# tobwei/APTAI

Measured on AMD Instinct MI355X. Metric: utterances/sec (10 s @ 16 kHz) train-step, higher is better.
Workload: dtype bf16

## Files before the change

### aptai_amd/csrc/common.h

```cpp
#pragma once
#include <hip/hip_runtime.h>
#include <stdint.h>
#include <stdio.h>
#include <string.h>

#include "../../include/aptai_hip.h"

typedef uint16_t bf16_t;

typedef __attribute__((ext_vector_type(8))) __bf16 bf16x8;
typedef __attribute__((ext_vector_type(4))) __bf16 bf16x4;
typedef __attribute__((ext_vector_type(4))) short short4v;
typedef __attribute__((ext_vector_type(8))) short short8v;
typedef __attribute__((ext_vector_type(4))) float f32x4;
typedef __attribute__((ext_vector_type(16))) float f32x16;
typedef __attribute__((ext_vector_type(2))) uint32_t u32x2;
typedef __attribute__((ext_vector_type(4))) uint32_t u32x4;

#define LDS_PTR(p) ((__attribute__((address_space(3))) void*)(p))
#define GLB_PTR(p) ((const __attribute__((address_space(1))) void*)(p))

void aptai_set_error(const char* fmt, ...);
const uint32_t* aptai_seed_salt(const void* stream);
const int32_t* aptai_frame_bounds(const void* stream);
#define APTAI_FAIL(code, ...)            \
    do {                                 \
        aptai_set_error(__VA_ARGS__);    \
        return (code);                   \
    } while (0)
#define APTAI_REQUIRE(cond, ...)                                   \
    do {                                                           \
        if (!(cond)) APTAI_FAIL(APTAI_ERR_INVALID, __VA_ARGS__);   \
    } while (0)
#define APTAI_LAUNCH(...)             \
    do {                              \
        (void)hipGetLastError();      \
        hipLaunchKernelGGL(__VA_ARGS__); \
    } while (0)
#define APTAI_CHECK_LAUNCH(name)                                                          \
    do {                                                                                  \
        hipError_t e__ = hipGetLastError();                                               \
        if (e__ != hipSuccess) APTAI_FAIL(APTAI_ERR_LAUNCH, "%s: %s", name, hipGetErrorString(e__)); \
    } while (0)

__device__ __forceinline__ float bf2f(bf16_t v) { return __uint_as_float(((uint32_t)v) << 16); }
__device__ __forceinline__ bf16_t f2bf(float f) {
    __bf16 b = (__bf16)f;
    return __builtin_bit_cast(bf16_t, b);
}
__device__ __forceinline__ uint32_t pack2bf(float lo, float hi) {
    typedef __bf16 bf2_t __attribute__((ext_vector_type(2)));
    typedef float f2_t __attribute__((ext_vector_type(2)));
    const f2_t v = {lo, hi};
    return __builtin_bit_cast(uint32_t, __builtin_convertvector(v, bf2_t));
}
__device__ __forceinline__ float lo_bf(uint32_t v) { return __uint_as_float(v << 16); }
__device__ __forceinline__ float hi_bf(uint32_t v) { return __uint_as_float(v & 0xffff0000u); }

__device__ __forceinline__ float wave_sum(float v) {
#pragma unroll
    for (int o = 32; o > 0; o >>= 1) v += __shfl_xor(v, o, 64);
    return v;
}
__device__ __forceinline__ float wave_max(float v) {
#pragma unroll
    for (int o = 32; o > 0; o >>= 1) v = fmaxf(v, __shfl_xor(v, o, 64));
    return v;
}

__device__ __forceinline__ float fast_exp2(float x) { return __builtin_amdgcn_exp2f(x); }
__device__ __forceinline__ float fast_log2(float x) { return __builtin_amdgcn_logf(x); }
__device__ __forceinline__ float gelu_erf(float x) { return 0.5f * x * (1.0f + erff(x * 0.70710678118654752f)); }
__device__ __forceinline__ float gelu_erf_grad(float x) {
    const float cdf = 0.5f * (1.0f + erff(x * 0.70710678118654752f));
    const float pdf = 0.39894228040143268f * __expf(-0.5f * x * x);
// ... 82 lines not shown
```

### aptai_amd/csrc/conv.hip

```cpp
#include <stdlib.h>

#include "common.h"

namespace {

constexpr int C0 = 512, KW = 10, STRIDE = 5;
constexpr int FRAMES_PER_BLOCK_STATS = 256;

struct Conv0Args {
    const float* audio; long S;
    const float* w; const float* bias; const float* gamma; const float* beta;
    bf16_t* out;
    int B, T_real, T_alloc;
    float eps;
    float* partials;
    const float* stats;
    int nchunks;
    const int* bounds;
};

__device__ __forceinline__ int frames_collated(const int* __restrict__ bounds, int T_real) {
    if (bounds == nullptr) return T_real;
    const int tb = bounds[0];
    return tb < 1 ? 1 : (tb < T_real ? tb : T_real);
// ... 95 lines not shown

template <bool LENS>
__global__ __launch_bounds__(256) void conv0_moments_kernel(const float* __restrict__ audio, long S, int T_static,
                                                            float* __restrict__ partials, int nch, const int* __restrict__ bounds,
                                                            const int* __restrict__ lens) {
    const int b = blockIdx.y, chunk = blockIdx.x;
    const int T_real = LENS ? frames_own(lens, b, bounds, T_static) : frames_collated(bounds, T_static);
    if (LENS && chunk * AC_FRAMES_PER_BLOCK >= T_real) return;
    __shared__ float red[4][AC_TERMS];
    const int lane = threadIdx.x & 63, wave = threadIdx.x >> 6;
    const float* xb = audio + (long)b * S;
    float acc[AC_TERMS];
#pragma unroll
    for (int i = 0; i < AC_TERMS; ++i) acc[i] = 0.f;
    const int t0 = chunk * AC_FRAMES_PER_BLOCK;
    int t1 = t0 + AC_FRAMES_PER_BLOCK;
    t1 = t1 < T_real ? t1 : T_real;
    for (int t = t0 + threadIdx.x; t < t1; t += 256) {
        float x[KW];
#pragma unroll
        for (int k = 0; k < KW; ++k) x[k] = xb[(long)t * STRIDE + k];
        int idx = KW;
#pragma unroll
        for (int k = 0; k < KW; ++k) {
            acc[k] += x[k];
#pragma unroll
            for (int k2 = k; k2 < KW; ++k2) { acc[idx] = fmaf(x[k], x[k2], acc[idx]); ++idx; }
        }
    }
#pragma unroll
    for (int i = 0; i < AC_TERMS; ++i) {
        const float v = wave_sum(acc[i]);
        if (lane == 0) red[wave][i] = v;
    }
    __syncthreads();
    if (threadIdx.x < AC_TERMS)
        partials[((long)b * nch + chunk) * AC_TERMS + threadIdx.x] =
            red[0][threadIdx.x] + red[1][threadIdx.x] + red[2][threadIdx.x] + red[3][threadIdx.x];
}

template <bool LENS>
__global__ void conv0_moments_final_kernel(const float* __restrict__ partials, const float* __restrict__ w,
                                           const float* __restrict__ bias, float* __restrict__ stats, int nch, int T_real,
                                           float eps, const int* __restrict__ bounds, const int* __restrict__ lens) {
    __shared__ double mom[AC_TERMS];
    const int b = blockIdx.x, c = threadIdx.x;
    const int frames = LENS ? frames_own(lens, b, bounds, T_real) : frames_collated(bounds, T_real);
    const int nsum = LENS ? (frames + AC_FRAMES_PER_BLOCK - 1) / AC_FRAMES_PER_BLOCK : nch;
    if (c < AC_TERMS) {
        double s = 0.0;
        for (int k = 0; k < nsum; ++k) s += (double)partials[((long)b * nch + k) * AC_TERMS + c];
        mom[c] = s / frames;
    }
    __syncthreads();
    double wk[KW];
#pragma unroll
    for (int k = 0; k < KW; ++k) wk[k] = (double)w[c * KW + k];
    const double bc = bias ? (double)bias[c] : 0.0;
    double wm = 0.0, q = 0.0;
    int idx = KW;
#pragma unroll
    for (int k = 0; k < KW; ++k) {
        wm += wk[k] * mom[k];
#pragma unroll
        for (int k2 = k; k2 < KW; ++k2) q += (k2 == k ? 1.0 : 2.0) * wk[k] * wk[k2] * mom[idx++];
    }
    const double mean = bc + wm;
    double var = q + 2.0 * bc * wm + bc * bc - mean * mean;
    var = var < 0.0 ? 0.0 : var;
    stats[((long)b * 2 + 0) * C0 + c] = (float)mean;
    stats[((long)b * 2 + 1) * C0 + c] = (float)(1.0 / sqrt(var + (double)eps));
}

typedef float f32x2 __attribute__((ext_vector_type(2)));

__device__ __forceinline__ f32x2 gelu_fast2(f32x2 x) {
    const f32x2 xc = {__builtin_amdgcn_fmed3f(x.x, -7.0f, 7.0f), __builtin_amdgcn_fmed3f(x.y, -7.0f, 7.0f)};
    const f32x2 x2 = xc * xc;
    f32x2 p = __builtin_elementwise_fma(x2, (f32x2){APTAI_GELU_A5 * APTAI_NLOG2E, APTAI_GELU_A5 * APTAI_NLOG2E},
                                        (f32x2){APTAI_GELU_A3 * APTAI_NLOG2E, APTAI_GELU_A3 * APTAI_NLOG2E});
    p = __builtin_elementwise_fma(p, x2, (f32x2){APTAI_GELU_A1 * APTAI_NLOG2E, APTAI_GELU_A1 * APTAI_NLOG2E});
    const f32x2 z = xc * p;
    const f32x2 e = (f32x2){__builtin_amdgcn_exp2f(z.x), __builtin_amdgcn_exp2f(z.y)} + (f32x2){1.0f, 1.0f};
    return x * (f32x2){__builtin_amdgcn_rcpf(e.x), __builtin_amdgcn_rcpf(e.y)};
}

template <bool LENS>
__global__ __launch_bounds__(256) void conv0_group_kernel(Conv0Args a, const int* __restrict__ lens) {
    const int lane = threadIdx.x & 63, wave = threadIdx.x >> 6;
    const int b = blockIdx.y;
    const int T_real = LENS ? frames_own(lens, b, a.bounds, a.T_real) : a.T_real;
    f32x2 w2[4][KW], b2[4];
    {
        float w[8][KW], bias[8];
        load_weights(a, lane, w, bias);
#pragma unroll
        for (int j = 0; j < 8; ++j) {
            const int c = lane * 8 + j;
            const float mu = a.stats[((long)b * 2 + 0) * C0 + c], rs = a.stats[((long)b * 2 + 1) * C0 + c];
            const float sc = rs * a.gamma[c];
            const float sh = fmaf(bias[j] - mu, sc, a.beta[c]);
#pragma unroll
            for (int k = 0; k < KW; ++k) w2[j >> 1][k][j & 1] = w[j][k] * sc;
            b2[j >> 1][j & 1] = sh;
        }
    }
// ... 612 lines not shown
        float v = t < T_real ? g[t * KW + r] : 0.f;
        if (t >= 1 && t - 1 < T_real) v += g[(t - 1) * KW + r + STRIDE];
        daudio[(long)b * S + s] = v;
    }
}

bool conv0_bwd_mfma() {
    static const bool on = !(getenv("APTAI_CONV0_BWD_MFMA") && atoi(getenv("APTAI_CONV0_BWD_MFMA")) == 0);
    return on;
}

}

extern "C" int64_t aptai_conv0_workspace_bytes(int64_t B, int64_t T_real) {
    const long nchunks = ceil_div(T_real, FRAMES_PER_BLOCK_STATS);
    return (B * nchunks * 2 * C0 + B * 2 * C0) * 4;
}

template <bool LENS>
static int conv0_fwd_impl(const char* who, const float* audio, int64_t B, int64_t S, const float* weight, const float* bias,
                          const float* gamma, const float* beta, int mode, float eps, void* out, int64_t T_real, int64_t T_alloc,
                          int64_t C, int64_t Kw, int64_t stride, void* workspace, float* stats_out, const int32_t* lens,
                          void* stream_) {
    hipStream_t stream = (hipStream_t)stream_;
    APTAI_REQUIRE(audio && weight && gamma && beta && out, "%s: null pointer", who);
    APTAI_REQUIRE(!LENS || lens, "%s: null frame_lens0", who);
    APTAI_REQUIRE(C == C0 && Kw == KW && stride == STRIDE, "%s: built for C=512, k=10, s=5 (got %ld,%ld,%ld)", who,
                  (long)C, (long)Kw, (long)stride);
    APTAI_REQUIRE(B > 0 && T_real > 0 && T_alloc >= T_real, "%s: bad frame counts", who);
    APTAI_REQUIRE((T_real - 1) * STRIDE + KW <= S, "%s: T_real=%ld frames need more than S=%ld samples", who, (long)T_real, (long)S);
    APTAI_REQUIRE(mode == 0 || mode == 1, "%s: mode must be 0 (group) or 1 (layer)", who);
    const int* bounds = (const int*)aptai_frame_bounds(stream_);
    Conv0Args a;
    memset(&a, 0, sizeof(a));
    a.audio = audio; a.S = S; a.w = weight; a.bias = bias; a.gamma = gamma; a.beta = beta;
    a.out = (bf16_t*)out; a.B = (int)B; a.T_real = (int)T_real; a.T_alloc = (int)T_alloc; a.eps = eps;
    if (LENS) a.bounds = bounds;
    long blocks = ceil_div(T_alloc, 4 * 8);
    if (blocks > 1024) blocks = 1024;
    if (mode == 1) {
        APTAI_LAUNCH(conv0_layer_kernel<LENS>, dim3((unsigned)blocks, (unsigned)B), dim3(256), 0, stream, a, (const int*)lens);
        APTAI_CHECK_LAUNCH("conv0_layer_kernel");
        return APTAI_OK;
    }
    APTAI_REQUIRE(workspace != nullptr, "%s: group mode needs a workspace", who);
    a.nchunks = (int)ceil_div(T_real, FRAMES_PER_BLOCK_STATS);
    a.partials = (float*)workspace;
    float* stats = stats_out ? stats_out : (float*)workspace + (long)B * a.nchunks * 2 * C0;
    a.stats = stats;
    const int nch = (int)ceil_div(T_real, AC_FRAMES_PER_BLOCK);
    APTAI_LAUNCH(conv0_moments_kernel<LENS>, dim3((unsigned)nch, (unsigned)B), dim3(256), 0, stream, audio, (long)S, (int)T_real,
                 a.partials, nch, bounds, (const int*)lens);
    APTAI_CHECK_LAUNCH("conv0_moments_kernel");
    APTAI_LAUNCH(conv0_moments_final_kernel<LENS>, dim3((unsigned)B), dim3(C0), 0, stream, (const float*)a.partials, weight, bias,
                 stats, nch, (int)T_real, eps, bounds, (const int*)lens);
    APTAI_CHECK_LAUNCH("conv0_moments_final_kernel");
    static int use_mfma = -1;
    if (use_mfma < 0) {
        const char* e = getenv("APTAI_CONV0_MFMA");
        use_mfma = e ? atoi(e) : 1;
    }
    if (use_mfma && T_alloc % 16 == 0) {
        long mb = ceil_div(1536, B);
        const long mb_max = ceil_div(T_alloc / 16, 4);
        if (mb > mb_max) mb = mb_max;
        APTAI_LAUNCH(conv0_group_mfma_kernel<LENS>, dim3((unsigned)mb, (unsigned)B), dim3(256), 0, stream, a, (const int*)lens);
        APTAI_CHECK_LAUNCH("conv0_group_mfma_kernel");
        return APTAI_OK;
    }
    APTAI_LAUNCH(conv0_group_kernel<LENS>, dim3((unsigned)blocks, (unsigned)B), dim3(256), 0, stream, a, (const int*)lens);
    APTAI_CHECK_LAUNCH("conv0_group_kernel");
    return APTAI_OK;
}

extern "C" int aptai_conv0_fwd(const float* audio, int64_t B, int64_t S, const float* weight, const float* bias,
                               const float* gamma, const float* beta, int mode, float eps, void* out, int64_t T_real,
                               int64_t T_alloc, int64_t C, int64_t Kw, int64_t stride, void* workspace, float* stats_out,
                               void* stream_) {
    return conv0_fwd_impl<false>("aptai_conv0_fwd", audio, B, S, weight, bias, gamma, beta, mode, eps, out, T_real, T_alloc, C, Kw, stride,
                                 workspace, stats_out, nullptr, stream_);
}

extern "C" int aptai_conv0_fwd_lens(const float* audio, int64_t B, int64_t S, const float* weight, const float* bias,
                                    const float* gamma, const float* beta, int mode, float eps, void* out, int64_t T_real,
                                    int64_t T_alloc, int64_t C, int64_t Kw, int64_t stride, void* workspace, float* stats_out,
                                    const int32_t* frame_lens0, void* stream_) {
    return conv0_fwd_impl<true>("aptai_conv0_fwd_lens", audio, B, S, weight, bias, gamma, beta, mode, eps, out, T_real, T_alloc, C, Kw,
                                stride, workspace, stats_out, frame_lens0, stream_);
}

extern "C" int64_t aptai_conv0_bwd_workspace_bytes(int64_t B, int64_t T_real) {
    const long nch = ceil_div(T_real, BWD_FRAMES_PER_BLOCK);
    return (B * nch * 2 * C0 + B * 2 * C0 + B * nch * C0 * 13) * 4;
}

extern "C" int aptai_conv0_bwd(const float* audio, int64_t B, int64_t S, const float* weight, const float* bias, const float* gamma,
                               const float* beta, int mode, float eps, const void* dy, int64_t T_real, int64_t T_alloc,
                               const float* fwd_stats, float* dweight, float* dbias, float* dgamma, float* dbeta, void* workspace,
                               void* stream_) {
    hipStream_t stream = (hipStream_t)stream_;
    APTAI_REQUIRE(audio && weight && gamma && beta && dy && dweight && workspace, "aptai_conv0_bwd: null pointer");
    APTAI_REQUIRE(mode == 0 || mode == 1, "aptai_conv0_bwd: mode");
    APTAI_REQUIRE(mode == 1 || fwd_stats, "aptai_conv0_bwd: group mode needs the forward statistics");
    APTAI_REQUIRE((T_real - 1) * STRIDE + KW <= S && T_alloc >= T_real, "aptai_conv0_bwd: bad frame counts");
    Conv0BwdArgs a;
    memset(&a, 0, sizeof(a));
    a.f.audio = audio; a.f.S = S; a.f.w = weight; a.f.bias = bias; a.f.gamma = gamma; a.f.beta = beta; a.f.B = (int)B;
    a.f.T_real = (int)T_real; a.f.T_alloc = (int)T_alloc; a.f.eps = eps; a.f.stats = fwd_stats;
// ... 76 lines not shown
```

### aptai_amd/csrc/elementwise.hip

```cpp
#include "common.h"

namespace {

__global__ void cast_f32_bf16_kernel(const float* __restrict__ src, bf16_t* __restrict__ dst, long n4) {
    const long stride = (long)gridDim.x * blockDim.x;
    for (long i = (long)blockIdx.x * blockDim.x + threadIdx.x; i < n4; i += stride) {
        const f32x4 v = ((const f32x4*)src)[i];
        ((u32x2*)dst)[i] = (u32x2){pack2bf(v[0], v[1]), pack2bf(v[2], v[3])};
    }
}

__global__ void cast_multi_kernel(const int64_t* __restrict__ table) {
    const int64_t* job = table + (long)blockIdx.y * 4;
    const long n = job[2];
    const long base = (long)blockIdx.x * 8192;
    if (base >= n) return;
    const float* src = (const float*)job[0];
    const bool copy = job[3] != 0;
#pragma unroll
    for (int it = 0; it < 4; ++it) {
        const long i = base + (long)(it * 256 + threadIdx.x) * 8;
        if (i >= n) break;
        const f32x4 a = *(const f32x4*)(src + i), b = *(const f32x4*)(src + i + 4);
        if (copy) {
// ... 88 lines not shown
        const int a = i / Kw, kk = i % Kw;
        const long src = dgrad ? (((long)(grp * Cg + a) * Cg + r) * Kw + kk) : ((long)row * n + i);
        slab[a * (Kw + 1) + kk] = v[src] * gain[kk] / norm[kk];
    }
    __syncthreads();
    bf16_t* out = (dgrad ? wd : wf) + (long)row * n;
    for (int j = threadIdx.x; j < n; j += 256) {
        const int kk = j / Cg, a = j % Cg;
        out[j] = f2bf(slab[a * (Kw + 1) + (dgrad ? Kw - 1 - kk : kk)]);
    }
}

__global__ __launch_bounds__(256) void posconv_wn_dot_kernel(const float* __restrict__ dwf, const float* __restrict__ v,
                                                             float* __restrict__ partial, int Cg, int Kw) {
    extern __shared__ float slab[];
    __shared__ float red[256];
    const int o = blockIdx.x, n = Cg * Kw;
    for (int i = threadIdx.x; i < n; i += 256) slab[(i / Cg) * (Cg + 1) + i % Cg] = dwf[(long)o * n + i];
    __syncthreads();
    float s = 0.f;
    for (int i = threadIdx.x; i < n; i += 256) {
        const int c = i / Kw, kk = i % Kw;
        s = fmaf(slab[kk * (Cg + 1) + c], v[(long)o * n + i], s);
    }
    red[threadIdx.x] = s;
    __syncthreads();
    if ((int)threadIdx.x < Kw) {
        float t = 0.f;
        for (int j = threadIdx.x; j < 256; j += Kw) t += red[j];
        partial[(long)o * Kw + threadIdx.x] = t;
    }
}
__global__ __launch_bounds__(256) void posconv_wn_final_kernel(const float* __restrict__ partial, const float* __restrict__ norm,
                                                               float* __restrict__ dot, float* __restrict__ dgain, int H, int Kw) {
    __shared__ float red[256];
    const int kk = blockIdx.x;
    const float s = tap_total(partial, H, Kw, kk, red);
    if (threadIdx.x == 0) {
        dot[kk] = s;
        dgain[kk] = s / norm[kk];
    }
}
__global__ __launch_bounds__(256) void posconv_wn_apply_kernel(const float* __restrict__ dwf, const float* __restrict__ v,
                                                               const float* __restrict__ gain, const float* __restrict__ norm,
                                                               const float* __restrict__ dot, float* __restrict__ dv, int Cg, int Kw) {
    extern __shared__ float slab[];
    const int o = blockIdx.x, n = Cg * Kw;
    for (int i = threadIdx.x; i < n; i += 256) slab[(i / Cg) * (Cg + 1) + i % Cg] = dwf[(long)o * n + i];
    __syncthreads();
    for (int i = threadIdx.x; i < n; i += 256) {
        const int c = i / Kw, kk = i % Kw;
        const float nr = norm[kk];
        dv[(long)o * n + i] = gain[kk] / nr * (slab[kk * (Cg + 1) + c] - v[(long)o * n + i] * dot[kk] / (nr * nr));
    }
}

__global__ void posconv_pack_kernel(const bf16_t* __restrict__ x, const bf16_t* __restrict__ u, bf16_t* __restrict__ xg,
                                    bf16_t* __restrict__ rowmajor_out, int B, int Tp, int H, int Cg, int pad) {
    const long n4 = (long)B * Tp * H / 4;
    const long stride = (long)gridDim.x * blockDim.x;
    const int G = H / Cg;
    const long rows_p = Tp + 2 * pad;
    for (long i = (long)blockIdx.x * blockDim.x + threadIdx.x; i < n4; i += stride) {
        const long e = i * 4;
        const long row = e / H;
        const int col = (int)(e % H);
        u32x2 p = *(const u32x2*)(x + e);
        if (u) {
            const u32x2 q = *(const u32x2*)(u + e);
            p = (u32x2){pack2bf(lo_bf(p[0]) * gelu_fast_grad(lo_bf(q[0])), hi_bf(p[0]) * gelu_fast_grad(hi_bf(q[0]))),
                        pack2bf(lo_bf(p[1]) * gelu_fast_grad(lo_bf(q[1])), hi_bf(p[1]) * gelu_fast_grad(hi_bf(q[1])))};
            if (rowmajor_out) *(u32x2*)(rowmajor_out + e) = p;
        }
        const int grp = col / Cg, c = col % Cg;
        const long b = row / Tp, t = row % Tp;
        *(u32x2*)(xg + (((long)grp * B + b) * rows_p + pad + t) * Cg + c) = p;
    }
    (void)G;
}

constexpr int SPEC_MAX_SPANS = 256;
__device__ __forceinline__ uint32_t spec_rand(uint32_t ctr, uint32_t s0, uint32_t s1) { return rng_hash(ctr * 2654435761u + 12345u, s0, s1); }

__global__ __launch_bounds__(64) void spec_mask_kernel(const int* __restrict__ lens, uint8_t* __restrict__ mask, int T, float mask_prob,
                                                       int mask_length, int min_masks, uint32_t s0, uint32_t s1,
                                                       const uint32_t* __restrict__ salt) {
    __shared__ int starts[SPEC_MAX_SPANS];
    __shared__ int nspan_sh;
    apply_salt(salt, s0, s1);
    const int b = blockIdx.x, lane = threadIdx.x;
    uint8_t* row = mask + (long)b * T;
    for (int t = lane; t < T; t += 64) row[t] = 0;
    int len = lens[b];
    len = len < 0 ? 0 : (len > T ? T : len);
    if (lane == 0) {
        const float eps = (float)(spec_rand(0xE951u, s0, s1) >> 8) * (1.0f / 16777216.0f);
        int n = (int)(mask_prob * (float)len / (float)mask_length + eps);
        n = n > min_masks ? n : min_masks;
        if (n * mask_length > T) n = T / mask_length;
        const int range = len - (mask_length - 1);
        if (range < n) n = range > 0 ? range : 0;
        n = n < SPEC_MAX_SPANS ? n : SPEC_MAX_SPANS;
        for (int i = 0; i < n; ++i) {
            const int j = range - n + i;
            const int t = (int)(spec_rand((uint32_t)(b * SPEC_MAX_SPANS + i + 1), s0, s1) % (uint32_t)(j + 1));
            bool taken = false;
// ... 212 lines not shown
        keep_scales8(i * 8, s0, s1, thr_tv, sc_tv, mt);
        keep_scales8(i * 8, s0 ^ 0x5bd1e995u, s1, thr_ph, sc_ph, mp);
#pragma unroll
        for (int r = 0; r < 8; ++r) {
            const float th = tanh_fast(x[r] * mt[r]);
            g[r] = gt[r] * (1.f - th * th) * mt[r] + gp[r] * (x[r] * mp[r] > 0.f ? 1.f : 0.01f) * mp[r];
        }
        *(u32x4*)(dh + i * 8) = pack8f(g);
    }
    for (long i = (n8 << 3) + (long)blockIdx.x * blockDim.x + threadIdx.x; i < n; i += stride) {
        const float x = bf2f(h[i]);
        float xt = x, xp = x, mt = 1.f, mp = 1.f;
        if (thr_tv) { mt = drop_keep((uint64_t)i, s0, s1, thr_tv) ? sc_tv : 0.f; xt = x * mt; }
        if (thr_ph) { mp = drop_keep((uint64_t)i, s0 ^ 0x5bd1e995u, s1, thr_ph) ? sc_ph : 0.f; xp = x * mp; }
        const float th = tanh_fast(xt);
        dh[i] = f2bf(bf2f(d_tv[i]) * (1.f - th * th) * mt + bf2f(d_ph[i]) * (xp > 0.f ? 1.f : 0.01f) * mp);
    }
}

__global__ void dropout_kernel(const bf16_t* __restrict__ x, bf16_t* __restrict__ y, long n, uint32_t s0, uint32_t s1,
                               uint32_t thr, float sc, const uint32_t* __restrict__ salt) {
    apply_salt(salt, s0, s1);
    const long stride = (long)gridDim.x * blockDim.x;
    const long n8 = n >> 3;
    for (long i = (long)blockIdx.x * blockDim.x + threadIdx.x; i < n8; i += stride) {
        float v[8], m[8];
        unpack8(*(const u32x4*)(x + i * 8), v);
        keep_scales8(i * 8, s0, s1, thr, sc, m);
#pragma unroll
        for (int r = 0; r < 8; ++r) v[r] *= m[r];
        *(u32x4*)(y + i * 8) = pack8f(v);
    }
    for (long i = (n8 << 3) + (long)blockIdx.x * blockDim.x + threadIdx.x; i < n; i += stride)
        y[i] = drop_keep((uint64_t)i, s0, s1, thr) ? f2bf(bf2f(x[i]) * sc) : (bf16_t)0;
}

__global__ void dgelu_kernel(const bf16_t* __restrict__ dy, const bf16_t* __restrict__ u, bf16_t* __restrict__ out, long n8) {
    const long stride = (long)gridDim.x * blockDim.x;
    for (long i = (long)blockIdx.x * blockDim.x + threadIdx.x; i < n8; i += stride) {
        const u32x4 d = ((const u32x4*)dy)[i], x = ((const u32x4*)u)[i];
        u32x4 o;
#pragma unroll
        for (int r = 0; r < 4; ++r)
            o[r] = pack2bf(lo_bf(d[r]) * gelu_fast_grad(lo_bf(x[r])), hi_bf(d[r]) * gelu_fast_grad(hi_bf(x[r])));
        ((u32x4*)out)[i] = o;
    }
}

inline unsigned grid_for(long n, int block = 256, int max_blocks = 4096) {
    long b = ceil_div(n, block);
    return (unsigned)(b < 1 ? 1 : (b > max_blocks ? max_blocks : b));
}

}

extern "C" int aptai_cast_f32_to_bf16(const float* src, void* dst, int64_t rows, int64_t cols, int64_t ld_dst, void* stream) {
    APTAI_REQUIRE(src && dst && rows > 0 && cols > 0, "aptai_cast_f32_to_bf16: bad arguments");
    if (ld_dst == cols && (rows * cols) % 4 == 0 && ((uintptr_t)src % 16 == 0) && ((uintptr_t)dst % 8 == 0)) {
        const long n4 = rows * cols / 4;
        APTAI_LAUNCH(cast_f32_bf16_kernel, dim3(grid_for(n4)), dim3(256), 0, (hipStream_t)stream, src, (bf16_t*)dst, n4);
    } else {
        APTAI_LAUNCH(cast_rows_kernel, dim3(grid_for(rows * cols)), dim3(256), 0, (hipStream_t)stream, src,
                           (bf16_t*)dst, (long)rows, (long)cols, (long)ld_dst);
    }
    APTAI_CHECK_LAUNCH("cast kernel");
    return APTAI_OK;
}

extern "C" int aptai_cast_multi(const int64_t* table_dev, int64_t njobs, int64_t max_n, void* stream) {
    APTAI_REQUIRE(table_dev && njobs > 0 && njobs <= 65535 && max_n > 0, "aptai_cast_multi: bad arguments");
    const long chunks = ceil_div(max_n, 8192);
    APTAI_LAUNCH(cast_multi_kernel, dim3((unsigned)chunks, (unsigned)njobs), dim3(256), 0, (hipStream_t)stream, table_dev);
    APTAI_CHECK_LAUNCH("cast_multi_kernel");
    return APTAI_OK;
}

extern "C" int aptai_conv_weight_to_bf16(const float* src, void* dst, int64_t N, int64_t C, int64_t Kw, void* stream) {
    APTAI_REQUIRE(src && dst && N > 0 && C > 0 && Kw > 0, "aptai_conv_weight_to_bf16: bad arguments");
    APTAI_LAUNCH(conv_weight_kernel, dim3(grid_for(N * C * Kw)), dim3(256), 0, (hipStream_t)stream, src, (bf16_t*)dst,
                       (int)N, (int)C, (int)Kw);
    APTAI_CHECK_LAUNCH("conv_weight_kernel");
    return APTAI_OK;
}

extern "C" int aptai_posconv_weight(const float* v, const float* gain, float* norm_ws, void* w_fwd, void* w_dgrad,
                                    int64_t H, int64_t groups, int64_t Kw, void* stream) {
    APTAI_REQUIRE(v && gain && norm_ws && w_fwd, "aptai_posconv_weight: null pointer");
    APTAI_REQUIRE(groups > 0 && H % groups == 0 && (H / groups) % 8 == 0, "aptai_posconv_weight: H=%ld groups=%ld", (long)H, (long)groups);
    const int Cg = (int)(H / groups);
    APTAI_REQUIRE(Kw > 0 && 256 % Kw == 0, "aptai_posconv_weight: Kw=%ld must divide 256", (long)Kw);
    const long nel = (long)H * Cg * Kw;
    float* partial = norm_ws + Kw;
    APTAI_LAUNCH(posconv_norm_partial_kernel, dim3(PCN_BLOCKS), dim3(256), 0, (hipStream_t)stream, v, partial, nel, (int)Kw);
    APTAI_CHECK_LAUNCH("posconv_norm_partial_kernel");
    APTAI_LAUNCH(posconv_norm_final_kernel, dim3((unsigned)Kw), dim3(256), 0, (hipStream_t)stream, (const float*)partial, norm_ws, (int)Kw);
    APTAI_CHECK_LAUNCH("posconv_norm_final_kernel");
    const size_t slab_bytes = (size_t)Cg * (Kw + 1) * 4;
    APTAI_REQUIRE(slab_bytes <= 64 * 1024, "aptai_posconv_weight: Cg*Kw slab of %ld bytes exceeds the LDS budget", (long)slab_bytes);
    APTAI_LAUNCH(posconv_weight_kernel, dim3((unsigned)(w_dgrad ? 2 * H : H)), dim3(256), slab_bytes, (hipStream_t)stream, v, gain,
                       (const float*)norm_ws, (bf16_t*)w_fwd, (bf16_t*)w_dgrad, (int)H, Cg, (int)Kw);
    APTAI_CHECK_LAUNCH("posconv_weight_kernel");
    return APTAI_OK;
}

extern "C" int aptai_spec_augment_mask(const int32_t* frame_lens, void* mask_u8, int64_t B, int64_t T, float mask_prob, int64_t mask_length,
                                       int64_t min_masks, uint64_t seed, void* stream) {
    APTAI_REQUIRE(frame_lens && mask_u8 && B > 0 && T > 0, "aptai_spec_augment_mask: bad arguments");
    APTAI_REQUIRE(mask_length >= 1 && mask_length <= T, "aptai_spec_augment_mask: mask_length=%ld must lie in [1, T=%ld]", (long)mask_length, (long)T);
    APTAI_REQUIRE(mask_prob >= 0.f && mask_prob <= 1.f && min_masks >= 0, "aptai_spec_augment_mask: bad mask_prob / min_masks");
    APTAI_LAUNCH(spec_mask_kernel, dim3((unsigned)B), dim3(64), 0, (hipStream_t)stream, frame_lens, (uint8_t*)mask_u8, (int)T, mask_prob,
                 (int)mask_length, (int)min_masks, (uint32_t)seed, (uint32_t)(seed >> 32), aptai_seed_salt(stream));
    APTAI_CHECK_LAUNCH("spec_mask_kernel");
    return APTAI_OK;
}

extern "C" int aptai_posconv_weight_bwd(const float* dw_fwd, const float* v, const float* gain, const float* norm, float* dv, float* dgain,
                                       float* workspace, int64_t H, int64_t groups, int64_t Kw, void* stream) {
    APTAI_REQUIRE(dw_fwd && v && gain && norm && dv && dgain && workspace, "aptai_posconv_weight_bwd: null pointer");
    APTAI_REQUIRE(groups > 0 && H % groups == 0 && Kw > 0 && 256 % Kw == 0, "aptai_posconv_weight_bwd: H=%ld groups=%ld Kw=%ld", (long)H, (long)groups, (long)Kw);
    const int Cg = (int)(H / groups);
    const size_t slab_bytes = (size_t)Kw * (Cg + 1) * 4;
    APTAI_REQUIRE(slab_bytes <= 64 * 1024, "aptai_posconv_weight_bwd: slab of %ld bytes exceeds the LDS budget", (long)slab_bytes);
    float* partial = workspace;
    float* dot = workspace + H * Kw;
    hipStream_t st = (hipStream_t)stream;
    APTAI_LAUNCH(posconv_wn_dot_kernel, dim3((unsigned)H), dim3(256), slab_bytes, st, dw_fwd, v, partial, Cg, (int)Kw);
    APTAI_CHECK_LAUNCH("posconv_wn_dot_kernel");
    APTAI_LAUNCH(posconv_wn_final_kernel, dim3((unsigned)Kw), dim3(256), 0, st, (const float*)partial, norm, dot, dgain, (int)H, (int)Kw);
    APTAI_CHECK_LAUNCH("posconv_wn_final_kernel");
    APTAI_LAUNCH(posconv_wn_apply_kernel, dim3((unsigned)H), dim3(256), slab_bytes, st, dw_fwd, v, gain, norm, (const float*)dot, dv, Cg, (int)Kw);
    APTAI_CHECK_LAUNCH("posconv_wn_apply_kernel");
    return APTAI_OK;
}

extern "C" int aptai_posconv_pack(const void* x, const void* u, void* xg, void* rowmajor_out, int64_t B, int64_t Tp,
                                  int64_t H, int64_t groups, int64_t pad, void* stream) {
    APTAI_REQUIRE(x && xg, "aptai_posconv_pack: null pointer");
    APTAI_REQUIRE(groups > 0 && H % groups == 0 && (H / groups) % 4 == 0, "aptai_posconv_pack: H=%ld groups=%ld", (long)H, (long)groups);
    APTAI_LAUNCH(posconv_pack_kernel, dim3(grid_for(B * Tp * H / 4)), dim3(256), 0, (hipStream_t)stream,
                       (const bf16_t*)x, (const bf16_t*)u, (bf16_t*)xg, (bf16_t*)rowmajor_out, (int)B, (int)Tp, (int)H,
                       (int)(H / groups), (int)pad);
    APTAI_CHECK_LAUNCH("posconv_pack_kernel");
    return APTAI_OK;
}

static int frame_mask_fwd_impl(const char* who, void* h, const int32_t* lens, const uint8_t* spec_mask, const float* embed,
                               const uint8_t* feat_mask, int64_t B, int64_t Tp, int64_t T, int64_t H, void* stream) {
    APTAI_REQUIRE(h && lens && H % 4 == 0, "%s: bad arguments", who);
    APTAI_REQUIRE(!spec_mask || embed, "%s: spec mask without masked_spec_embed", who);
    APTAI_REQUIRE((uintptr_t)feat_mask % 4 == 0, "%s: feat_mask must be 4-byte aligned", who);
    const dim3 grid(grid_for(B * Tp * H / 4));
    if (feat_mask)
        APTAI_LAUNCH(frame_mask_kernel<true>, grid, dim3(256), 0, (hipStream_t)stream, (bf16_t*)h, lens, spec_mask, embed, feat_mask,
                     (int)B, (int)Tp, (int)T, (int)H);
    else
        APTAI_LAUNCH(frame_mask_kernel<false>, grid, dim3(256), 0, (hipStream_t)stream, (bf16_t*)h, lens, spec_mask, embed, feat_mask,
                     (int)B, (int)Tp, (int)T, (int)H);
    APTAI_CHECK_LAUNCH("frame_mask_kernel");
    return APTAI_OK;
}
extern "C" int aptai_frame_mask_fwd(void* h, const int32_t* lens, const uint8_t* spec_mask, const float* embed, int64_t B,
                                    int64_t Tp, int64_t T, int64_t H, void* stream) {
    return frame_mask_fwd_impl("aptai_frame_mask_fwd", h, lens, spec_mask, embed, nullptr, B, Tp, T, H, stream);
}
extern "C" int aptai_frame_feature_mask_fwd(void* h, const int32_t* lens, const uint8_t* spec_mask, const float* embed,
                                            const uint8_t* feat_mask, int64_t B, int64_t Tp, int64_t T, int64_t H, void* stream) {
    return frame_mask_fwd_impl("aptai_frame_feature_mask_fwd", h, lens, spec_mask, embed, feat_mask, B, Tp, T, H, stream);
}

static const int MASK_BWD_RPB = 32;
extern "C" int64_t aptai_frame_mask_bwd_workspace_bytes(int64_t B, int64_t Tp, int64_t H) {
    return ceil_div(B * Tp, MASK_BWD_RPB) * H * 4;
}
static int frame_mask_bwd_impl(const char* who, void* dy, const int32_t* lens, const uint8_t* spec_mask, const uint8_t* feat_mask,
                               float* dembed, void* workspace, int64_t B, int64_t Tp, int64_t T, int64_t H, void* stream) {
    APTAI_REQUIRE(dy && lens && H % 4 == 0, "%s: bad arguments", who);
    APTAI_REQUIRE((uintptr_t)feat_mask % 4 == 0, "%s: feat_mask must be 4-byte aligned", who);
    const long blocks = ceil_div(B * Tp, MASK_BWD_RPB);
    const bool want = spec_mask && dembed;
    APTAI_REQUIRE(!want || workspace, "%s: workspace needed for dembed", who);
    float* partials = want ? (float*)workspace : nullptr;
    if (feat_mask)
        APTAI_LAUNCH(frame_mask_bwd_kernel<true>, dim3((unsigned)blocks), dim3(256), 0, (hipStream_t)stream, (bf16_t*)dy, lens,
// ... 79 lines not shown
```

### aptai_amd/csrc/posconv.hip

```cpp
#include "common.h"

namespace {

constexpr int CG = 48, KW = 128, FR = 128;
constexpr int KTOT = KW * CG;
constexpr int XROWS = FR + KW - 1;
constexpr int X_BYTES = 6 * 256 * 16;
constexpr int W_STAGE = 512 * 16;

struct PosconvArgs {
    const bf16_t* xg; long x_group_stride, x_batch_stride;
    const bf16_t* w;
    const float* bias;
    const bf16_t* residual;
    bf16_t* out;
    bf16_t* out_pre;
    int Tp, H, gelu;
};

__device__ __forceinline__ void posconv_store(const PosconvArgs& a, const f32x4 accv, long row, int col) {
    float v[4] = {accv[0], accv[1], accv[2], accv[3]};
    if (a.bias) {
        const f32x4 bv = *(const f32x4*)(a.bias + col);
#pragma unroll
// ... 36 lines not shown
    }
    auto stage_w = [&](char* buf) {
#pragma unroll
        for (int it = 0; it < 2; ++it) {
            __builtin_amdgcn_global_load_lds(GLB_PTR(pw[it]), LDS_PTR(buf + (it * 256 + wave * 64) * 16), 16, 0, 0);
            pw[it] += 64;
        }
    };
    stage_w(sW);

    f32x4 acc[2][3];
#pragma unroll
    for (int i = 0; i < 2; ++i)
#pragma unroll
        for (int j = 0; j < 3; ++j) acc[i][j] = (f32x4){0.f, 0.f, 0.f, 0.f};

    const int a_off = (wave * 32 + (lane & 15)) * (CG * 2) + (lane >> 4) * 16;
    int b_off[3][2];
#pragma unroll
    for (int j = 0; j < 3; ++j)
#pragma unroll
        for (int ks = 0; ks < 2; ++ks) {
            const int row = j * 16 + (lane & 15), q = ks * 4 + (lane >> 4);
            b_off[j][ks] = row * 128 + ((q ^ (row & 7)) << 4);
        }

    constexpr int NKT = KTOT / 64;
    for (int kt = 0; kt < NKT; ++kt) {
        asm volatile("s_waitcnt vmcnt(0)" ::: "memory");
        __syncthreads();
        const int cur = kt & 1;
        if (kt + 1 < NKT) stage_w(sW + (cur ^ 1) * W_STAGE);
        const char* sw = sW + cur * W_STAGE;
        const char* sa = sX + a_off + kt * 128;
        bf16x8 af[2][2], bfr[2][3];
#pragma unroll
        for (int ks = 0; ks < 2; ++ks) {
#pragma unroll
            for (int i = 0; i < 2; ++i) af[ks][i] = *(const bf16x8*)(sa + i * (16 * CG * 2) + ks * 64);
#pragma unroll
            for (int j = 0; j < 3; ++j) bfr[ks][j] = *(const bf16x8*)(sw + b_off[j][ks]);
        }
#pragma unroll
        for (int ks = 0; ks < 2; ++ks)
#pragma unroll
            for (int i = 0; i < 2; ++i)
#pragma unroll
                for (int j = 0; j < 3; ++j)
                    acc[i][j] = __builtin_amdgcn_mfma_f32_16x16x32_bf16(bfr[ks][j], af[ks][i], acc[i][j], 0, 0, 0);
    }
#pragma unroll
    for (int i = 0; i < 2; ++i) {
        const long row = (long)b * a.Tp + t0 + wave * 32 + i * 16 + (lane & 15);
#pragma unroll
        for (int j = 0; j < 3; ++j) posconv_store(a, acc[i][j], row, grp * CG + j * 16 + (lane >> 4) * 4);
    }
}

constexpr int CG2 = 64, PITCH2 = 144;
constexpr int X2_BYTES = (XROWS + 1) * PITCH2;
constexpr int W2_STAGE = CG2 * 128;

__global__ __launch_bounds__(256, 3) void posconv64_kernel(PosconvArgs a) {
    extern __shared__ __attribute__((aligned(16))) char smem[];
    char* sX = smem;
    char* sW = smem + X2_BYTES;
    const int tid = threadIdx.x, lane = tid & 63;
    const int wave = __builtin_amdgcn_readfirstlane(tid >> 6);
    const int t0 = blockIdx.x * FR, b = blockIdx.y, grp = blockIdx.z;
    const bf16_t* xsrc = a.xg + (long)grp * a.x_group_stride + (long)b * a.x_batch_stride + (long)t0 * CG2;
    for (int c = tid; c < XROWS * 8; c += 256) {
        const int fr = c >> 3, ch = c & 7;
        *(u32x4*)(sX + fr * PITCH2 + ch * 16) = *(const u32x4*)(xsrc + (long)fr * CG2 + ch * 8);
    }
    const bf16_t* wg = a.w + (long)grp * CG2 * (KW * CG2);
    const bf16_t* pw[2];
#pragma unroll
    for (int it = 0; it < 2; ++it) {
        const int c = it * 256 + tid, row = c >> 3, pc = c & 7;
        pw[it] = wg + (long)row * (KW * CG2) + ((pc ^ (row & 7)) << 3);
    }
    auto stage_w = [&](char* buf) {
#pragma unroll
        for (int it = 0; it < 2; ++it) {
            __builtin_amdgcn_global_load_lds(GLB_PTR(pw[it]), LDS_PTR(buf + (it * 256 + wave * 64) * 16), 16, 0, 0);
            pw[it] += 64;
        }
    };
    stage_w(sW);
    f32x4 acc[2][4];
#pragma unroll
    for (int i = 0; i < 2; ++i)
#pragma unroll
        for (int j = 0; j < 4; ++j) acc[i][j] = (f32x4){0.f, 0.f, 0.f, 0.f};
    const int a_off = (wave * 32 + (lane & 15)) * PITCH2 + (lane >> 4) * 16;
    int b_off[4][2];
#pragma unroll
    for (int j = 0; j < 4; ++j)
#pragma unroll
        for (int ks = 0; ks < 2; ++ks) {
            const int row = j * 16 + (lane & 15), q = ks * 4 + (lane >> 4);
            b_off[j][ks] = row * 128 + ((q ^ (row & 7)) << 4);
        }
    for (int kt = 0; kt < KW; ++kt) {
        asm volatile("s_waitcnt vmcnt(0)" ::: "memory");
        __syncthreads();
// ... 114 lines not shown
                    acc[i][j] = __builtin_amdgcn_mfma_f32_16x16x32_bf16(bfr[j], af[i], acc[i][j], 0, 0, 0);
        }
    }
    float* out = a.dw + (long)grp * CG * KTOT;
#pragma unroll
    for (int i = 0; i < 3; ++i) {
        const int m = i * 16 + (lane & 15);
#pragma unroll
        for (int j = 0; j < 2; ++j) {
            const int n = n0 + wave * 32 + j * 16 + (lane >> 4) * 4;
            *(f32x4*)(out + (long)m * KTOT + n) = acc[i][j];
        }
    }
}

}

extern "C" int aptai_posconv_wgrad(const void* du_g, const void* x_g, float* dw, int64_t B, int64_t Tp, int64_t H, int64_t groups,
                                   int64_t Kw, int64_t pad, void* stream) {
    APTAI_REQUIRE(du_g && x_g && dw, "aptai_posconv_wgrad: null pointer");
    APTAI_REQUIRE(groups > 0 && H == groups * CG && Kw == KW && 2 * pad == KW, "aptai_posconv_wgrad: built for 48 channels per group, 128 taps, pad 64");
    const long rows_p = Tp + 2 * pad;
    const long frames = B * rows_p - 2 * pad;
    APTAI_REQUIRE(B > 0 && Tp > 0 && frames % 64 == 0, "aptai_posconv_wgrad: %ld frames per group is not a multiple of 64", (long)frames);
    PosconvWgradArgs a;
    a.du = (const bf16_t*)du_g + pad * CG;
    a.x = (const bf16_t*)x_g;
    a.group_stride = B * rows_p * CG;
    a.dw = dw;
    a.nkt = (int)(frames / 64);
    APTAI_LAUNCH(posconv_wgrad_kernel, dim3((unsigned)(KTOT / WG_NT), (unsigned)groups), dim3(256), 2 * WG_STAGE, (hipStream_t)stream, a);
    APTAI_CHECK_LAUNCH("posconv_wgrad_kernel");
    return APTAI_OK;
}

extern "C" int aptai_posconv_gemm(const void* xg, int64_t first_row, const void* w, const float* bias, const void* residual, void* out,
                                  void* out_pre, int64_t B, int64_t Tp, int64_t H, int64_t groups, int64_t Kw, int64_t pad, int gelu,
                                  void* stream) {
    APTAI_REQUIRE(xg && w && out, "aptai_posconv_gemm: null pointer");
    APTAI_REQUIRE(groups > 0 && (H == groups * CG || H == groups * CG2) && Kw == KW,
                  "aptai_posconv_gemm: built for 48 or 64 channels per group and 128 taps (H=%ld groups=%ld Kw=%ld)", (long)H, (long)groups, (long)Kw);
    APTAI_REQUIRE(B > 0 && Tp > 0 && Tp % FR == 0, "aptai_posconv_gemm: Tp=%ld must be a positive multiple of %d", (long)Tp, FR);
    APTAI_REQUIRE(first_row >= 0 && first_row + KW - 1 <= 2 * pad, "aptai_posconv_gemm: first_row=%ld leaves the padded window (pad=%ld)",
                  (long)first_row, (long)pad);
    const long cg = H / groups;
    const long rows_p = Tp + 2 * pad;
    PosconvArgs a;
    a.xg = (const bf16_t*)xg + first_row * cg;
    a.x_batch_stride = rows_p * cg;
    a.x_group_stride = B * rows_p * cg;
    a.w = (const bf16_t*)w; a.bias = bias; a.residual = (const bf16_t*)residual; a.out = (bf16_t*)out; a.out_pre = (bf16_t*)out_pre;
    a.Tp = (int)Tp; a.H = (int)H; a.gelu = gelu;
    const dim3 grid((unsigned)(Tp / FR), (unsigned)B, (unsigned)groups);
    if (cg == CG) APTAI_LAUNCH(posconv_kernel, grid, dim3(256), X_BYTES + 2 * W_STAGE, (hipStream_t)stream, a);
    else APTAI_LAUNCH(posconv64_kernel, grid, dim3(256), X2_BYTES + 2 * W2_STAGE, (hipStream_t)stream, a);
    APTAI_CHECK_LAUNCH("posconv_kernel");
    return APTAI_OK;
}
```

### aptai_amd/csrc/runtime.hip

```cpp
#include <stdarg.h>

#include "common.h"

static thread_local char g_err[512] = "";

void aptai_set_error(const char* fmt, ...) {
    va_list ap;
    va_start(ap, fmt);
    vsnprintf(g_err, sizeof(g_err), fmt, ap);
    va_end(ap);
}

extern "C" const char* aptai_last_error(void) { return g_err; }
extern "C" int aptai_version(void) { return 100; }

extern "C" int aptai_device_check(char* name, int name_len) {
    int dev = 0;
    if (hipGetDevice(&dev) != hipSuccess) APTAI_FAIL(APTAI_ERR_NO_DEVICE, "no HIP device is current");
    hipDeviceProp_t prop;
    if (hipGetDeviceProperties(&prop, dev) != hipSuccess) APTAI_FAIL(APTAI_ERR_NO_DEVICE, "hipGetDeviceProperties failed");
    if (name && name_len > 0) {
        strncpy(name, prop.gcnArchName, (size_t)name_len - 1);
        name[name_len - 1] = 0;
    }
    if (strncmp(prop.gcnArchName, "gfx950", 6) != 0)
        APTAI_FAIL(APTAI_ERR_NO_DEVICE, "device is %s; this library is built for gfx950 only", prop.gcnArchName);
    return APTAI_OK;
}

#include <mutex>
namespace {
constexpr int SALT_SLOTS = 64;
struct SaltSlot { const void* stream; const uint32_t* ptr; bool used; };
SaltSlot g_salts[SALT_SLOTS];
std::mutex g_salt_mu;
}

extern "C" int aptai_set_seed_salt(void* stream, const void* device_ptr_2xu32) {
    std::lock_guard<std::mutex> lk(g_salt_mu);
    int free_slot = -1;
    for (int i = 0; i < SALT_SLOTS; ++i) {
        if (g_salts[i].used && g_salts[i].stream == stream) {
            if (device_ptr_2xu32) g_salts[i].ptr = (const uint32_t*)device_ptr_2xu32;
            else g_salts[i].used = false;
            return APTAI_OK;
        }
        if (!g_salts[i].used && free_slot < 0) free_slot = i;
    }
    if (!device_ptr_2xu32) return APTAI_OK;
    if (free_slot < 0) APTAI_FAIL(APTAI_ERR_INVALID, "aptai_set_seed_salt: more than %d streams carry a salt", SALT_SLOTS);
    g_salts[free_slot] = {stream, (const uint32_t*)device_ptr_2xu32, true};
    return APTAI_OK;
}
const uint32_t* aptai_seed_salt(const void* stream) {
    std::lock_guard<std::mutex> lk(g_salt_mu);
    for (int i = 0; i < SALT_SLOTS; ++i)
        if (g_salts[i].used && g_salts[i].stream == stream) return g_salts[i].ptr;
    return nullptr;
}


namespace {
SaltSlot g_bounds[SALT_SLOTS];
// ... 25 lines not shown
```

Measured before the change: 1756.

## Add wide variants of posconv, weight-norm and conv0 moment kernels

```diff
diff --git a/aptai_amd/csrc/common.h b/aptai_amd/csrc/common.h
--- a/aptai_amd/csrc/common.h
+++ b/aptai_amd/csrc/common.h
@@ -21,6 +21,7 @@
 #define GLB_PTR(p) ((const __attribute__((address_space(1))) void*)(p))
 
 void aptai_set_error(const char* fmt, ...);
+bool aptai_front_wide();
 const uint32_t* aptai_seed_salt(const void* stream);
 const int32_t* aptai_frame_bounds(const void* stream);
 #define APTAI_FAIL(code, ...)            \
diff --git a/aptai_amd/csrc/conv.hip b/aptai_amd/csrc/conv.hip
--- a/aptai_amd/csrc/conv.hip
+++ b/aptai_amd/csrc/conv.hip
@@ -171,6 +171,48 @@
         for (int k = 0; k < nsum; ++k) s += (double)partials[((long)b * nch + k) * AC_TERMS + c];
         mom[c] = s / frames;
     }
+    __syncthreads();
+    double wk[KW];
+#pragma unroll
+    for (int k = 0; k < KW; ++k) wk[k] = (double)w[c * KW + k];
+    const double bc = bias ? (double)bias[c] : 0.0;
+    double wm = 0.0, q = 0.0;
+    int idx = KW;
+#pragma unroll
+    for (int k = 0; k < KW; ++k) {
+        wm += wk[k] * mom[k];
+#pragma unroll
+        for (int k2 = k; k2 < KW; ++k2) q += (k2 == k ? 1.0 : 2.0) * wk[k] * wk[k2] * mom[idx++];
+    }
+    const double mean = bc + wm;
+    double var = q + 2.0 * bc * wm + bc * bc - mean * mean;
+    var = var < 0.0 ? 0.0 : var;
+    stats[((long)b * 2 + 0) * C0 + c] = (float)mean;
+    stats[((long)b * 2 + 1) * C0 + c] = (float)(1.0 / sqrt(var + (double)eps));
+}
+
+constexpr int AC_FINAL_TILE = 64;
+
+template <bool LENS>
+__global__ void conv0_moments_final_wide_kernel(const float* __restrict__ partials, const float* __restrict__ w,
+                                                const float* __restrict__ bias, float* __restrict__ stats, int nch, int T_real,
+                                                float eps, const int* __restrict__ bounds, const int* __restrict__ lens) {
+    __shared__ double mom[AC_TERMS];
+    __shared__ float pl[AC_FINAL_TILE * AC_TERMS];
+    const int b = blockIdx.x, c = threadIdx.x;
+    const int frames = LENS ? frames_own(lens, b, bounds, T_real) : frames_collated(bounds, T_real);
+    const int nsum = LENS ? (frames + AC_FRAMES_PER_BLOCK - 1) / AC_FRAMES_PER_BLOCK : nch;
+    double s = 0.0;
+    for (int k0 = 0; k0 < nsum; k0 += AC_FINAL_TILE) {
+        const int n = nsum - k0 < AC_FINAL_TILE ? nsum - k0 : AC_FINAL_TILE;
+        const float* src = partials + ((long)b * nch + k0) * AC_TERMS;
+        for (int i = threadIdx.x; i < n * AC_TERMS; i += C0) pl[i] = src[i];
+        __syncthreads();
+        if (c < AC_TERMS)
+            for (int k = 0; k < n; ++k) s += (double)pl[k * AC_TERMS + c];
+        __syncthreads();
+    }
+    if (c < AC_TERMS) mom[c] = s / frames;
     __syncthreads();
     double wk[KW];
 #pragma unroll
@@ -889,8 +931,12 @@
     APTAI_LAUNCH(conv0_moments_kernel<LENS>, dim3((unsigned)nch, (unsigned)B), dim3(256), 0, stream, audio, (long)S, (int)T_real,
                  a.partials, nch, bounds, (const int*)lens);
     APTAI_CHECK_LAUNCH("conv0_moments_kernel");
-    APTAI_LAUNCH(conv0_moments_final_kernel<LENS>, dim3((unsigned)B), dim3(C0), 0, stream, (const float*)a.partials, weight, bias,
-                 stats, nch, (int)T_real, eps, bounds, (const int*)lens);
+    if (aptai_front_wide())
+        APTAI_LAUNCH(conv0_moments_final_wide_kernel<LENS>, dim3((unsigned)B), dim3(C0), 0, stream, (const float*)a.partials, weight, bias,
+                     stats, nch, (int)T_real, eps, bounds, (const int*)lens);
+    else
+        APTAI_LAUNCH(conv0_moments_final_kernel<LENS>, dim3((unsigned)B), dim3(C0), 0, stream, (const float*)a.partials, weight, bias,
+                     stats, nch, (int)T_real, eps, bounds, (const int*)lens);
     APTAI_CHECK_LAUNCH("conv0_moments_final_kernel");
     static int use_mfma = -1;
     if (use_mfma < 0) {
diff --git a/aptai_amd/csrc/elementwise.hip b/aptai_amd/csrc/elementwise.hip
--- a/aptai_amd/csrc/elementwise.hip
+++ b/aptai_amd/csrc/elementwise.hip
@@ -164,6 +164,86 @@
         const int c = i / Kw, kk = i % Kw;
         const float nr = norm[kk];
         dv[(long)o * n + i] = gain[kk] / nr * (slab[kk * (Cg + 1) + c] - v[(long)o * n + i] * dot[kk] / (nr * nr));
+    }
+}
+
+__global__ __launch_bounds__(256) void posconv_weight_wide_kernel(const float* __restrict__ v, const float* __restrict__ gain,
+                                                                  const float* __restrict__ norm, bf16_t* __restrict__ wf,
+                                                                  bf16_t* __restrict__ wd, int H, int Cg, int Kw) {
+    extern __shared__ float slab[];
+    const bool dgrad = (int)blockIdx.x >= H;
+    const int row = dgrad ? blockIdx.x - H : blockIdx.x;
+    const int grp = row / Cg, r = row % Cg;
+    const int n = Cg * Kw;
+#pragma unroll 6
+    for (int i = threadIdx.x * 4; i < n; i += 1024) {
+        const int a = i / Kw, kk = i % Kw;
+        const long src = dgrad ? (((long)(grp * Cg + a) * Cg + r) * Kw + kk) : ((long)row * n + i);
+        const f32x4 x = *(const f32x4*)(v + src), g = *(const f32x4*)(gain + kk), nr = *(const f32x4*)(norm + kk);
+#pragma unroll
+        for (int e = 0; e < 4; ++e) slab[a * (Kw + 1) + kk + e] = x[e] * g[e] / nr[e];
+    }
+    __syncthreads();
+    bf16_t* out = (dgrad ? wd : wf) + (long)row * n;
+    for (int j = threadIdx.x * 8; j < n; j += 2048) {
+        const int kk = j / Cg, a = j % Cg;
+        const float* s = slab + a * (Kw + 1) + (dgrad ? Kw - 1 - kk : kk);
+        *(u32x4*)(out + j) = (u32x4){pack2bf(s[0], s[Kw + 1]), pack2bf(s[2 * (Kw + 1)], s[3 * (Kw + 1)]),
+                                     pack2bf(s[4 * (Kw + 1)], s[5 * (Kw + 1)]), pack2bf(s[6 * (Kw + 1)], s[7 * (Kw + 1)])};
+    }
+}
+
+__global__ __launch_bounds__(256) void posconv_wn_dot_wide_kernel(const float* __restrict__ dwf, const float* __restrict__ v,
+                                                                  float* __restrict__ partial, int Cg, int Kw) {
+    extern __shared__ __attribute__((aligned(16))) float wslab[];
+    __shared__ float red[256];
+    const int o = blockIdx.x, n = Cg * Kw;
+    float* vrow = wslab + Kw * (Cg + 1);
+#pragma unroll 6
+    for (int i = threadIdx.x * 4; i < n; i += 1024) {
+        const f32x4 d = *(const f32x4*)(dwf + (long)o * n + i);
+        *(f32x4*)(vrow + i) = *(const f32x4*)(v + (long)o * n + i);
+        float* s = wslab + (i / Cg) * (Cg + 1) + i % Cg;
+#pragma unroll
+        for (int e = 0; e < 4; ++e) s[e] = d[e];
+    }
+    __syncthreads();
+    float s = 0.f;
+    for (int i = threadIdx.x; i < n; i += 256) {
+        const int c = i / Kw, kk = i % Kw;
+        s = fmaf(wslab[kk * (Cg + 1) + c], vrow[i], s);
+    }
+    red[threadIdx.x] = s;
+    __syncthreads();
+    if ((int)threadIdx.x < Kw) {
+        float t = 0.f;
+        for (int j = threadIdx.x; j < 256; j += Kw) t += red[j];
+        partial[(long)o * Kw + threadIdx.x] = t;
+    }
+}
+
+__global__ __launch_bounds__(256) void posconv_wn_apply_wide_kernel(const float* __restrict__ dwf, const float* __restrict__ v,
+                                                                    const float* __restrict__ gain, const float* __restrict__ norm,
+                                                                    const float* __restrict__ dot, float* __restrict__ dv, int Cg, int Kw) {
+    extern __shared__ __attribute__((aligned(16))) float wslab[];
+    const int o = blockIdx.x, n = Cg * Kw;
+#pragma unroll 6
+    for (int i = threadIdx.x * 4; i < n; i += 1024) {
+        const f32x4 d = *(const f32x4*)(dwf + (long)o * n + i);
+        float* s = wslab + (i / Cg) * (Cg + 1) + i % Cg;
+#pragma unroll
+        for (int e = 0; e < 4; ++e) s[e] = d[e];
+    }
+    __syncthreads();
+#pragma unroll 6
+    for (int i = threadIdx.x * 4; i < n; i += 1024) {
+        const int c = i / Kw, kk = i % Kw;
+        const f32x4 x = *(const f32x4*)(v + (long)o * n + i), g = *(const f32x4*)(gain + kk), nr = *(const f32x4*)(norm + kk),
+                    dt = *(const f32x4*)(dot + kk);
+        f32x4 r;
+#pragma unroll
+        for (int e = 0; e < 4; ++e) r[e] = g[e] / nr[e] * (wslab[(kk + e) * (Cg + 1) + c] - x[e] * dt[e] / (nr[e] * nr[e]));
+        *(f32x4*)(dv + (long)o * n + i) = r;
     }
 }
 
@@ -482,6 +562,9 @@
     return (unsigned)(b < 1 ? 1 : (b > max_blocks ? max_blocks : b));
 }
 
+template <class... P>
+inline bool aligned16(const P*... p) { return (((uintptr_t)p | ...) & 15) == 0; }
+
 }
 
 extern "C" int aptai_cast_f32_to_bf16(const float* src, void* dst, int64_t rows, int64_t cols, int64_t ld_dst, void* stream) {
@@ -527,8 +610,12 @@
     APTAI_CHECK_LAUNCH("posconv_norm_final_kernel");
     const size_t slab_bytes = (size_t)Cg * (Kw + 1) * 4;
     APTAI_REQUIRE(slab_bytes <= 64 * 1024, "aptai_posconv_weight: Cg*Kw slab of %ld bytes exceeds the LDS budget", (long)slab_bytes);
-    APTAI_LAUNCH(posconv_weight_kernel, dim3((unsigned)(w_dgrad ? 2 * H : H)), dim3(256), slab_bytes, (hipStream_t)stream, v, gain,
-                       (const float*)norm_ws, (bf16_t*)w_fwd, (bf16_t*)w_dgrad, (int)H, Cg, (int)Kw);
+    if (aptai_front_wide() && Kw % 4 == 0 && aligned16(v, gain, norm_ws, w_fwd, w_dgrad))
+        APTAI_LAUNCH(posconv_weight_wide_kernel, dim3((unsigned)(w_dgrad ? 2 * H : H)), dim3(256), slab_bytes, (hipStream_t)stream, v, gain,
+                     (const float*)norm_ws, (bf16_t*)w_fwd, (bf16_t*)w_dgrad, (int)H, Cg, (int)Kw);
+    else
+        APTAI_LAUNCH(posconv_weight_kernel, dim3((unsigned)(w_dgrad ? 2 * H : H)), dim3(256), slab_bytes, (hipStream_t)stream, v, gain,
+                     (const float*)norm_ws, (bf16_t*)w_fwd, (bf16_t*)w_dgrad, (int)H, Cg, (int)Kw);
     APTAI_CHECK_LAUNCH("posconv_weight_kernel");
     return APTAI_OK;
 }
@@ -554,11 +641,19 @@
     float* partial = workspace;
     float* dot = workspace + H * Kw;
     hipStream_t st = (hipStream_t)stream;
-    APTAI_LAUNCH(posconv_wn_dot_kernel, dim3((unsigned)H), dim3(256), slab_bytes, st, dw_fwd, v, partial, Cg, (int)Kw);
+    const bool wide = aptai_front_wide() && Kw % 4 == 0 && Cg % 4 == 0 && aligned16(dw_fwd, v, gain, norm, dv, workspace);
+    const size_t dot_bytes = slab_bytes + (size_t)Cg * Kw * 4;
+    if (wide && dot_bytes <= 64 * 1024)
+        APTAI_LAUNCH(posconv_wn_dot_wide_kernel, dim3((unsigned)H), dim3(256), dot_bytes, st, dw_fwd, v, partial, Cg, (int)Kw);
+    else
+        APTAI_LAUNCH(posconv_wn_dot_kernel, dim3((unsigned)H), dim3(256), slab_bytes, st, dw_fwd, v, partial, Cg, (int)Kw);
     APTAI_CHECK_LAUNCH("posconv_wn_dot_kernel");
     APTAI_LAUNCH(posconv_wn_final_kernel, dim3((unsigned)Kw), dim3(256), 0, st, (const float*)partial, norm, dot, dgain, (int)H, (int)Kw);
     APTAI_CHECK_LAUNCH("posconv_wn_final_kernel");
-    APTAI_LAUNCH(posconv_wn_apply_kernel, dim3((unsigned)H), dim3(256), slab_bytes, st, dw_fwd, v, gain, norm, (const float*)dot, dv, Cg, (int)Kw);
+    if (wide)
+        APTAI_LAUNCH(posconv_wn_apply_wide_kernel, dim3((unsigned)H), dim3(256), slab_bytes, st, dw_fwd, v, gain, norm, (const float*)dot, dv, Cg, (int)Kw);
+    else
+        APTAI_LAUNCH(posconv_wn_apply_kernel, dim3((unsigned)H), dim3(256), slab_bytes, st, dw_fwd, v, gain, norm, (const float*)dot, dv, Cg, (int)Kw);
     APTAI_CHECK_LAUNCH("posconv_wn_apply_kernel");
     return APTAI_OK;
 }
diff --git a/aptai_amd/csrc/posconv.hip b/aptai_amd/csrc/posconv.hip
--- a/aptai_amd/csrc/posconv.hip
+++ b/aptai_amd/csrc/posconv.hip
@@ -112,6 +112,97 @@
 #pragma unroll
     for (int i = 0; i < 2; ++i) {
         const long row = (long)b * a.Tp + t0 + wave * 32 + i * 16 + (lane & 15);
+#pragma unroll
+        for (int j = 0; j < 3; ++j) posconv_store(a, acc[i][j], row, grp * CG + j * 16 + (lane >> 4) * 4);
+    }
+}
+
+constexpr int FRW = 256;
+constexpr int XW_CHUNKS = (FRW + KW - 1) * CG * 2 / 16;
+constexpr int XW_IT = (XW_CHUNKS + 255) / 256;
+constexpr int XW_BYTES = XW_IT * 256 * 16;
+
+__global__ __launch_bounds__(256, 3) void posconv_wide_kernel(PosconvArgs a) {
+    extern __shared__ __attribute__((aligned(16))) char smem[];
+    char* sX = smem;
+    char* sW = smem + XW_BYTES;
+    const int tid = threadIdx.x, lane = tid & 63;
+    const int wave = __builtin_amdgcn_readfirstlane(tid >> 6);
+    const int t0 = blockIdx.x * FRW, b = blockIdx.y, grp = blockIdx.z;
+    const bool half = a.Tp - t0 < FRW;
+    const bool idle = half && wave >= 2;
+
+    const bf16_t* xsrc = a.xg + (long)grp * a.x_group_stride + (long)b * a.x_batch_stride + (long)t0 * CG;
+    const int xlast = (half ? XROWS * CG * 2 / 16 : XW_CHUNKS) - 1;
+#pragma unroll
+    for (int it = 0; it < XW_IT; ++it) {
+        int c = it * 256 + tid;
+        c = c < xlast ? c : xlast;
+        __builtin_amdgcn_global_load_lds(GLB_PTR(xsrc + (long)c * 8), LDS_PTR(sX + (it * 256 + wave * 64) * 16), 16, 0, 0);
+    }
+    const bf16_t* wg = a.w + (long)grp * CG * KTOT;
+    const bf16_t* pw[2];
+#pragma unroll
+    for (int it = 0; it < 2; ++it) {
+        const int c = it * 256 + tid, row = c >> 3, pc = c & 7;
+        const int r = row < CG ? row : CG - 1;
+        pw[it] = wg + (long)r * KTOT + ((pc ^ (row & 7)) << 3);
+    }
+    auto stage_w = [&](char* buf) {
+#pragma unroll
+        for (int it = 0; it < 2; ++it) {
+            __builtin_amdgcn_global_load_lds(GLB_PTR(pw[it]), LDS_PTR(buf + (it * 256 + wave * 64) * 16), 16, 0, 0);
+            pw[it] += 64;
+        }
+    };
+    stage_w(sW);
+
+    f32x4 acc[4][3];
+#pragma unroll
+    for (int i = 0; i < 4; ++i)
+#pragma unroll
+        for (int j = 0; j < 3; ++j) acc[i][j] = (f32x4){0.f, 0.f, 0.f, 0.f};
+
+    const int a_off = (wave * 64 + (lane & 15)) * (CG * 2) + (lane >> 4) * 16;
+    int b_off[3][2];
+#pragma unroll
+    for (int j = 0; j < 3; ++j)
+#pragma unroll
+        for (int ks = 0; ks < 2; ++ks) {
+            const int row = j * 16 + (lane & 15), q = ks * 4 + (lane >> 4);
+            b_off[j][ks] = row * 128 + ((q ^ (row & 7)) << 4);
+        }
+
+    constexpr int NKT = KTOT / 64;
+    for (int kt = 0; kt < NKT; ++kt) {
+        asm volatile("s_waitcnt vmcnt(0)" ::: "memory");
+        __syncthreads();
+        const int cur = kt & 1;
+        if (kt + 1 < NKT) stage_w(sW + (cur ^ 1) * W_STAGE);
+        if (idle) continue;
+        const char* sw = sW + cur * W_STAGE;
+        const char* sa = sX + a_off + kt * 128;
+        bf16x8 af[2][4], bfr[2][3];
+#pragma unroll
+        for (int ks = 0; ks < 2; ++ks) {
+#pragma unroll
+            for (int j = 0; j < 3; ++j) bfr[ks][j] = *(const bf16x8*)(sw + b_off[j][ks]);
+#pragma unroll
+            for (int i = 0; i < 4; ++i) af[ks][i] = *(const bf16x8*)(sa + i * (16 * CG * 2) + ks * 64);
+        }
+        __builtin_amdgcn_sched_barrier(0);
+#pragma unroll
+        for (int ks = 0; ks < 2; ++ks)
+#pragma unroll
+            for (int i = 0; i < 4; ++i)
+#pragma unroll
+                for (int j = 0; j < 3; ++j)
+                    acc[i][j] = __builtin_amdgcn_mfma_f32_16x16x32_bf16(bfr[ks][j], af[ks][i], acc[i][j], 0, 0, 0);
+    }
+    if (idle) return;
+#pragma unroll
+    for (int i = 0; i < 4; ++i) {
+        const long row = (long)b * a.Tp + t0 + wave * 64 + i * 16 + (lane & 15);
 #pragma unroll
         for (int j = 0; j < 3; ++j) posconv_store(a, acc[i][j], row, grp * CG + j * 16 + (lane >> 4) * 4);
     }
@@ -332,7 +423,10 @@
     a.w = (const bf16_t*)w; a.bias = bias; a.residual = (const bf16_t*)residual; a.out = (bf16_t*)out; a.out_pre = (bf16_t*)out_pre;
     a.Tp = (int)Tp; a.H = (int)H; a.gelu = gelu;
     const dim3 grid((unsigned)(Tp / FR), (unsigned)B, (unsigned)groups);
-    if (cg == CG) APTAI_LAUNCH(posconv_kernel, grid, dim3(256), X_BYTES + 2 * W_STAGE, (hipStream_t)stream, a);
+    if (cg == CG && aptai_front_wide()) {
+        const dim3 wide((unsigned)((Tp + FRW - 1) / FRW), (unsigned)B, (unsigned)groups);
+        APTAI_LAUNCH(posconv_wide_kernel, wide, dim3(256), XW_BYTES + 2 * W_STAGE, (hipStream_t)stream, a);
+    } else if (cg == CG) APTAI_LAUNCH(posconv_kernel, grid, dim3(256), X_BYTES + 2 * W_STAGE, (hipStream_t)stream, a);
     else APTAI_LAUNCH(posconv64_kernel, grid, dim3(256), X2_BYTES + 2 * W2_STAGE, (hipStream_t)stream, a);
     APTAI_CHECK_LAUNCH("posconv_kernel");
     return APTAI_OK;
diff --git a/aptai_amd/csrc/runtime.hip b/aptai_amd/csrc/runtime.hip
--- a/aptai_amd/csrc/runtime.hip
+++ b/aptai_amd/csrc/runtime.hip
@@ -9,6 +9,11 @@
     va_start(ap, fmt);
     vsnprintf(g_err, sizeof(g_err), fmt, ap);
     va_end(ap);
+}
+
+bool aptai_front_wide() {
+    static const bool on = !(getenv("APTAI_FRONT_WIDE") && atoi(getenv("APTAI_FRONT_WIDE")) == 0);
+    return on;
 }
 
 extern "C" const char* aptai_last_error(void) { return g_err; }
```

New measurement: 1763 (median of 6 runs). Within noise of the previous version (+0.4%).
